# Draghoyns/FLAIR-1

Measured on AMD Instinct MI355X. Metric: 512x512x5 tiles/s (train fwd+bwd), higher is better.
Workload: dtype bf16; 1 GPU; U-Net/ResNet34 5-ch 512x512 13-class train step (fwd + fused CE/argmax/confmat + bwd + SGD), bs=32/GPU, random-init weights; global_batch=32, parallelism=dp1, grad_allreduce=none

## Files before the change

flair-1_amd/csrc/capi.hip:

```cpp
#include <new>
#include <string.h>

#include "../../include/flair_hip.h"
#include "unet.h"
#include "conv_args.h"
#include "parity_pack.h"
#include "segformer.h"
#include "upernet.h"
#include "segformer_ops.h"
#include "swin_ops.h"

using namespace flair;

struct flair_unet { UNet net; flair_unet(int a, int b, int c) : net(a, b, c) {} };
struct flair_segformer {
  SegFormer net;
  flair_segformer(int a, int b, const int* d, const int* h, const int* hd, const int* sr, int dh, int dt) : net(a, b, d, h, hd, sr, dh, dt) {}
};

struct flair_upernet {
  UperNet net;
  flair_upernet(int a, int b, int e, const int* d, const int* h, int hid, const int* ps, int ai, int ac, int dt)
      : net(a, b, e, d, h, hid, ps, ai, ac, dt) {}
};
// ... 605 lines not shown
  if (dtype != DT_F32 && dtype != DT_BF16) return -2;
  return maxpool3x3s2_bwd(dtype, dy, idx, dx, accumulate, N, H, W, C, (hipStream_t)stream, bnr_y, bnr_msc, bnr_msh, bnr_partial);
}
int flair_bn_act(int dtype, const void* y, const float* scale, const float* shift, void* out, int64_t rows, int C, int relu, void* stream) {
  if (!y || !scale || !shift || !out || rows < 1 || C < 1) return -1;
  if (dtype != DT_F32 && dtype != DT_BF16) return -2;
  return bn_act(dtype, y, scale, shift, nullptr, nullptr, nullptr, out, (long)rows, C, relu, (hipStream_t)stream);
}
int flair_bn_act_maxpool(int dtype, const void* y, const float* scale, const float* shift, void* act, void* out, uint8_t* idx, int N,
                         int H, int W, int C, void* stream) {
  if (!y || !scale || !shift || !act || !out || N < 1 || H < 1 || W < 1 || C < 1) return -1;
  if (dtype != DT_F32 && dtype != DT_BF16) return -2;
  return bn_act_maxpool3x3s2(dtype, y, scale, shift, act, out, idx, N, H, W, C, (hipStream_t)stream);
}
int flair_upcat_bwd(int dtype, const void* dcat, void* dx0, int dx0_accumulate, void* dskip, int dskip_accumulate, int N, int H, int W,
                    int C0, int C1, void* stream) {
  if (!dcat || !dx0 || (C1 > 0 && !dskip) || N < 1 || H < 1 || W < 1 || C0 < 1 || C1 < 0) return -1;
  if (dtype != DT_F32 && dtype != DT_BF16) return -2;
  return upcat_bwd(dtype, dcat, dx0, dx0_accumulate, dskip, dskip_accumulate, N, H, W, C0, C1, (hipStream_t)stream);
}
int flair_ew_add(int dtype, void* dst, const void* src, int64_t n, void* stream) {
  if (!dst || !src || n < 1) return -1;
  if (dtype != DT_F32 && dtype != DT_BF16) return -2;
  return ew_add(dtype, dst, src, (long)n, (hipStream_t)stream);
}
int flair_colsum(int dtype, const void* x, int64_t rows, int ld, int C, float* out, void* workspace, size_t wsb, void* stream) {
  if (!x || !out || !workspace || rows < 1 || ld < 1 || C < 1) return -1;
  if (dtype != DT_F32 && dtype != DT_BF16) return -2;
  OpArena ar(workspace, wsb);
  float* partial = (float*)ar.get((size_t)bn_bwd_blocks((long)rows) * ld * 4);
  if (ar.bad) return -100;
  return colsum(dtype, x, (long)rows, ld, C, partial, out, (hipStream_t)stream);
}
int flair_pack_weights(int dtype, const float* params, const flair_pack_desc_t* descs, int n, void* base, void* stream) {
  if (!params || !descs || !base) return -1;
  if ((dtype != DT_F32 && dtype != DT_BF16) || n < 1 || n > PackTable::MAX) return -2;
  PackTable tb;
  tb.n = n;
  for (int i = 0; i < n; ++i) {
    const flair_pack_desc_t& q = descs[i];
    const int taps = q.Rc > 0 ? q.Rc * q.Sc : q.R * q.S;
    if (q.Cout < 1 || q.Cin < 1 || q.R < 1 || q.S < 1 || taps < 1 || (long)taps * q.Cin_p > q.Kpad || q.Cin_p < (q.tf ? q.Cout : q.Cin) ||
        q.rows_pad < (q.tf ? q.Cin : q.Cout) || q.w_off < 0)
      return -2;
    const bool vec = dtype == DT_BF16 && q.R * q.S == 9 &&
                     (q.tf ? ((q.Cin & 31) == 0 && (q.Cout & 31) == 0) : (q.Rc == 0 && (q.Cin & 3) == 0));
    if (vec && (((uintptr_t)params & 15) || (q.w_off & 3))) return -2;
    if (q.Rc > 0 && (q.r0 + (q.Rc - 1) * q.rstep >= q.R || q.s0 + (q.Sc - 1) * q.sstep >= q.S || q.r0 < 0 || q.s0 < 0 || q.rstep < 1 || q.sstep < 1))
      return -2;
    PackDesc& d = tb.d[i];
    memset(&d, 0, sizeof(d));
    d.w_off = (long)q.w_off; d.dst_off = (size_t)q.dst_off; d.Cout = q.Cout; d.Cin = q.Cin; d.R = q.R; d.S = q.S;
    d.Cin_p = q.Cin_p; d.rows_pad = q.rows_pad; d.Kpad = q.Kpad; d.tf = q.tf;
    d.r0 = (unsigned char)q.r0; d.rstep = (unsigned char)q.rstep; d.Rc = (unsigned char)q.Rc;
    d.s0 = (unsigned char)q.s0; d.sstep = (unsigned char)q.sstep; d.Sc = (unsigned char)q.Sc;
  }
  return pack_weights_all(dtype, params, base, tb, (hipStream_t)stream);
}
int flair_pack_weight(int dtype, const float* w_oihw, void* dst, int Cout, int Cin, int R, int S, int Cin_p, int rows_pad, int Kpad,
                      int tf, void* stream) {
  if (!w_oihw || !dst) return -1;
  if (dtype != DT_F32 && dtype != DT_BF16) return -2;
  if (Cout < 1 || Cin < 1 || R < 1 || S < 1 || (long)R * S * Cin_p > Kpad || Cin_p < (tf ? Cout : Cin) || rows_pad < (tf ? Cin : Cout))
    return -2;
  return pack_weight(dtype, w_oihw, dst, Cout, Cin, R, S, Cin_p, rows_pad, Kpad, tf ? 1 : 0, (hipStream_t)stream);
}

int flair_maxpool_forward(int dtype, const void* x, void* y, uint8_t* idx, int N, int H, int W, int C, void* stream) {
  return maxpool3x3s2_fwd(dtype, x, y, idx, N, H, W, C, (hipStream_t)stream);
}
int flair_maxpool_backward(int dtype, const void* dy, const uint8_t* idx, void* dx, int N, int H, int W, int C, void* stream) {
  return maxpool3x3s2_bwd(dtype, dy, idx, dx, 0, N, H, W, C, (hipStream_t)stream);
}
int flair_nchw_to_nhwc(int dtype, const float* x, void* y, int N, int C, int H, int W, int Cpad, void* stream) {
  return nchw_f32_to_nhwc(dtype, x, y, N, C, H, W, Cpad, (hipStream_t)stream);
}
int flair_nhwc_to_nchw(int dtype, const void* x, float* y, int N, int C, int H, int W, int Cpad, void* stream) {
  return nhwc_to_nchw_f32(dtype, x, y, N, C, H, W, Cpad, nullptr, (hipStream_t)stream);
}

#define FLAIR_DT_OK(dt) ((dt) == DT_F32 || (dt) == DT_BF16)
int flair_sf_layernorm(int dtype, const void* x, const float* gamma, const float* beta, void* y, int64_t rows, int C, float eps, void* stream) {
  if (!x || !gamma || !beta || !y || rows < 1 || C < 1) return -1;
  if (!FLAIR_DT_OK(dtype)) return -2;
  return sf_layernorm(dtype, x, gamma, beta, y, (long)rows, C, eps, (hipStream_t)stream);
}
int flair_sf_dwconv3x3_gelu(int dtype, const void* x, const float* w, const float* bias, void* y, int B, int H, int W, int C, void* stream) {
  if (!x || !w || !bias || !y || B < 1 || H < 1 || W < 1 || C < 1) return -1;
  if (!FLAIR_DT_OK(dtype)) return -2;
  return sf_dwconv3x3_gelu(dtype, x, w, bias, y, B, H, W, C, (hipStream_t)stream);
// ... 165 lines not shown
```

flair-1_amd/csrc/misc.hip:

```cpp
#include "ops.h"
#include "prof.h"

namespace flair {

static inline int ew_blocks(long total) {
  long b = (total + 255) / 256;
  if (b > 256 * 16) b = 256 * 16;
  if (b < 1) b = 1;
  return (int)b;
}

template <typename T>
__global__ void maxpool_fwd_kernel(const T* __restrict__ in, T* __restrict__ out, unsigned char* __restrict__ idx,
                                   int N, int H, int W, int C) {
  constexpr int CH = Elem<T>::CH;
  const int Ho = H / 2, Wo = W / 2, cpr = C / CH;
  const int ho = blockIdx.x % Ho, n = blockIdx.x / Ho;
  const unsigned row_items = (unsigned)Wo * cpr;
  for (unsigned it = threadIdx.x; it < row_items; it += blockDim.x) {
    const int cx = (int)(it % (unsigned)cpr), wo = (int)(it / (unsigned)cpr);
    const long i = ((long)blockIdx.x * Wo + wo) * cpr + cx;
    float best[CH];
    unsigned char bi[CH];
#pragma unroll
// ... 338 lines not shown
        }
      }
      __syncthreads();
      for (int e = t; e < 32 * 32 * RSc; e += 256) {
        const int kk = e & 31, rest = e >> 5;
        const int tp = rest % RSc, cc = rest / RSc;
        if (k0 + kk < d.Cout && c0 + cc < d.Cin) {
          const int r = r0 + (tp / Sc) * rstep, q = s0 + (tp % Sc) * sstep;
          const float v = tile[(kk * 32 + cc) * RS + (d.R - 1 - r) * d.S + (d.S - 1 - q) + (kk >> 3)];
          dst[(long)(c0 + cc) * d.Kpad + tp * d.Cin_p + k0 + kk] = Elem<T>::from_f(v);
        }
      }
    }
  } else {
    const long total = (long)d.Cin * d.Cout * RSc;
    for (long i = (long)blockIdx.x * 256 + t; i < total; i += (long)gridDim.x * 256) {
      const int k = (int)(i % d.Cout);
      const long rest = i / d.Cout;
      const int tp = (int)(rest % RSc), c = (int)(rest / RSc);
      const int r = r0 + (tp / Sc) * rstep, q = s0 + (tp % Sc) * sstep;
      dst[(long)c * d.Kpad + tp * d.Cin_p + k] =
          Elem<T>::from_f(w[(((long)k * d.Cin + c) * d.R + (d.R - 1 - r)) * d.S + (d.S - 1 - q)]);
    }
  }
  const int nrows = d.tf ? d.Cin : d.Cout, ncols = d.tf ? d.Cout : d.Cin;
  const long total = (long)d.rows_pad * d.Kpad;
  for (long i = (long)blockIdx.x * 256 + t; i < total; i += (long)gridDim.x * 256) {
    const int row = (int)(i / d.Kpad), kk = (int)(i - (long)row * d.Kpad);
    const int tp = kk / d.Cin_p, c = kk - tp * d.Cin_p;
    if (row >= nrows || tp >= RSc || c >= ncols) dst[i] = Elem<T>::from_f(0.f);
  }
}

int pack_weights_all(int dtype, const float* params, void* base, const PackTable& tb, hipStream_t s) {
  if (tb.n < 1 || tb.n > PackTable::MAX) return -2;
  double bytes = 0;
  for (int i = 0; i < tb.n; ++i) bytes += (double)tb.d[i].Cout * tb.d[i].Cin * tb.d[i].R * tb.d[i].S * 4.0 + (double)tb.d[i].rows_pad * tb.d[i].Kpad * dtype_size(dtype);
  ProfScope ps("pack_weights_all", 0.0, bytes, s);
  dim3 grid(256, tb.n);
  if (dtype == DT_F32)
    hipLaunchKernelGGL(pack_weights_all_kernel<float>, grid, dim3(256), 0, s, params, (unsigned char*)base, tb);
  else
    hipLaunchKernelGGL(pack_weights_all_kernel<bf16_t>, grid, dim3(256), 0, s, params, (unsigned char*)base, tb);
  FLAIR_CHECK_LAUNCH();
  return 0;
}

__global__ void sgd_kernel(float* __restrict__ p, const float* __restrict__ g, long n, float lr) {
  const long n4 = n / 4;
  for (long i = (long)blockIdx.x * blockDim.x + threadIdx.x; i < n4; i += (long)gridDim.x * blockDim.x) {
    float4 a = reinterpret_cast<float4*>(p)[i];
    const float4 b = reinterpret_cast<const float4*>(g)[i];
    a.x -= lr * b.x; a.y -= lr * b.y; a.z -= lr * b.z; a.w -= lr * b.w;
    reinterpret_cast<float4*>(p)[i] = a;
  }
  if (blockIdx.x == 0 && threadIdx.x < (n & 3)) {
    const long i = n4 * 4 + threadIdx.x;
    p[i] -= lr * g[i];
  }
}

__global__ void add_rowvec_kernel(float* __restrict__ x, const float* __restrict__ v, int N, int C, int H, int W) {
  const long total = (long)N * C * H * W;
  for (long i = (long)blockIdx.x * blockDim.x + threadIdx.x; i < total; i += (long)gridDim.x * blockDim.x) {
    const int h = (int)((i / W) % H);
    const int n = (int)(i / ((long)C * H * W));
    x[i] += v[n * H + h];
  }
}

template <typename T>
__global__ void add_rowvec_nhwc_kernel(T* __restrict__ x, const float* __restrict__ v, long nchunks, int row_chunks) {
  constexpr int CH = Elem<T>::CH;
  for (long i = (long)blockIdx.x * blockDim.x + threadIdx.x; i < nchunks; i += (long)gridDim.x * blockDim.x) {
    const float a = v[i / row_chunks];
    float f[CH];
// ... 236 lines not shown
```

flair-1_amd/csrc/ops.h:

```cpp
#pragma once
#include "common.h"
#include "conv_route.h"

namespace flair {

int bn_finalize(const float* partial, int nblk, int C, long count, const float* gamma, const float* beta,
                float* running_mean, float* running_var, float momentum, float eps, float* scale, float* shift,
                float* mean_out, float* invstd_out, hipStream_t s);
int bn_eval_coeffs(int C, const float* gamma, const float* beta, const float* rm, const float* rv, float eps,
                   float* scale, float* shift, hipStream_t s);
int bn_act(int dtype, const void* y, const float* scale, const float* shift, const void* res, const float* rscale,
           const float* rshift, void* out, long rows, int C, int relu, hipStream_t s);
int bn_bwd_blocks(long rows);
int bn_backward(int dtype, const void* dout, const void* out, const void* y, const float* mean, const float* invstd,
                const float* gamma, long rows, int C, float* partial, float* coef, float* dgamma, float* dbeta,
                int accumulate_param, void* dy, void* dres, int dres_accumulate, const float* mscale, const float* mshift,
                int pre_nblk ,
                int premasked , hipStream_t s);

int partial_rows_sum(const float* partial, int nblk, int ncols, float* out, hipStream_t s);
int bn_stats_partial(int dtype, const void* y, long rows, int C, float* partial, float* zeros_ones, hipStream_t s);
int colsum(int dtype, const void* x, long rows, int ld, int C, float* partial, float* out, hipStream_t s);

int maxpool3x3s2_fwd(int dtype, const void* in, void* out, unsigned char* idx, int N, int H, int W, int C, hipStream_t s);
int bn_act_maxpool3x3s2(int dtype, const void* y, const float* scale, const float* shift, void* act, void* out, unsigned char* idx, int N, int H,
                        int W, int C, hipStream_t s);
int maxpool3x3s2_bwd(int dtype, const void* dout, const unsigned char* idx, void* din, int accumulate, int N, int H,
                     int W, int C, hipStream_t s, const void* bnr_y = nullptr, const float* bnr_msc = nullptr,
                     const float* bnr_msh = nullptr, float* bnr_partial = nullptr);
int upcat_bwd(int dtype, const void* dcat, void* dx0, int dx0_accumulate, void* dskip, int dskip_accumulate, int N,
              int H, int W, int C0, int C1, hipStream_t s);
int nchw_f32_to_nhwc(int dtype, const float* in, void* out, int N, int C, int H, int W, int Cp, hipStream_t s);
int nhwc_to_nchw_f32(int dtype, const void* in, float* out, int N, int C, int H, int W, int Cp, float* accumulate_into,
                     hipStream_t s);
int pack_weight(int dtype, const float* w_oihw, void* dst, int Cout, int Cin, int R, int S, int Cin_p, int rows_pad,
                int Kpad, int transpose_flip, hipStream_t s);
struct PackDesc {
  long w_off;
  size_t dst_off;
  int Cout, Cin, R, S, Cin_p, rows_pad, Kpad, tf;
  unsigned char r0, rstep, Rc, s0, sstep, Sc, pad_[2];
};
inline PackDesc pack_desc(long w_off, size_t dst_off, int Cout, int Cin, int R, int Cin_p, int rows_pad, int Kpad, int tf) {
  PackDesc d = {};
  d.w_off = w_off; d.dst_off = dst_off; d.Cout = Cout; d.Cin = Cin; d.R = R; d.S = R;
  d.Cin_p = Cin_p; d.rows_pad = rows_pad; d.Kpad = Kpad; d.tf = tf;
  return d;
}
struct PackTable {
  static constexpr int MAX = 64;
  int n;
  PackDesc d[MAX];
};
int pack_weights_all(int dtype, const float* params, void* base, const PackTable& tb, hipStream_t s);
int sgd_step(float* params, const float* grads, long n, float lr, hipStream_t s);
int add_rowvec_nchw(float* x, const float* v, int N, int C, int H, int W, hipStream_t s);
int add_rowvec_nhwc(int dtype, void* x, const float* v, int N, int H, int W, int C, hipStream_t s);
int add_rowvec_nhwc_to(int dtype, const void* x, const float* v, void* y, int N, int H, int W, int C, hipStream_t s);
int rowvec_grad_nhwc(int dtype, const void* dx, float* dv, int N, int H, int W, int C, hipStream_t s);
int ew_add(int dtype, void* dst, const void* src, long n, hipStream_t s);
int fill_zero(void* p, size_t bytes, hipStream_t s);
int fill_f32(float* p, long n, float v, hipStream_t s);

struct CeArgs {
  const float* logits;
  const void* logits_nhwc = nullptr;
  int logits_dtype = 0, logits_ld = 0;
  const void* labels;
  int label_kind;
  const float* weight;
  int B, C, H, W;
  float* loss;
  float* dlogits_nchw;
  void* dlogits_nhwc;
  int dlogits_dtype, dlogits_ld;
  unsigned char* preds_u8;
  long long* preds_i64;
  int* targets_i32;
  long long* confmat;
  float* workspace;
};
size_t ce_workspace_floats(int B, int H, int W);
int ce_head(const CeArgs& a, hipStream_t s);
constexpr int CE_MAX_BLOCKS = 2048;
struct CeWorkspace { unsigned char* lab8; float* den_partial; float* loss_partial; float* den; };
CeWorkspace ce_workspace_layout(float* workspace, long npix);
int ce_labels(const void* labels, int label_kind, const float* weight, int B, int C, int H, int W, int* targets_i32, float* workspace, hipStream_t s);
int ce_finish(float* workspace, long npix, int nblk, float* loss, hipStream_t s);
// ... 42 lines not shown
```

flair-1_amd/csrc/unet.h:

```cpp
#pragma once
#include <string>
#include <vector>

#include "ops.h"

namespace flair {

struct Act {
  void* p = nullptr;
  int N = 0, H = 0, W = 0, C = 0;
  const float* lz_scale = nullptr;
  const float* lz_shift = nullptr;
  long rows() const { return (long)N * H * W; }
  long elems() const { return rows() * C; }
};

struct ConvDesc {
  std::string name;
  int Cin, Cout, R, S, stride, pad;
  int Cin_p, Cout_p;
  bool bias;
  long w_off = -1, b_off = -1;
  size_t wf = 0, wd = 0;
  int Kpad, rows_f;
// ... 113 lines not shown
  std::vector<hipEvent_t> fork_ev_;
  hipEvent_t join_ev_ = nullptr;
  size_t fork_next_ = 0;
  bool side_pending_ = false;
  Act f5m_;
  float* drows_pending_ = nullptr;
  bool side_init();
  hipStream_t wgrad_stream();
  int side_cus() const;
  void side_join();
 public:
  ~UNet();
 private:
  void* dl_nhwc_ = nullptr;
  void* logits_nhwc_ = nullptr;
  void* const* stage_events_ = nullptr;
  void stage_done(int stage);

  struct GradBuf { void* act; void* g; bool init; };
  int sole_producer(const Act& a) const;
  int residual_producer(const Act& a) const;
  void attach_bn_reduce(ConvArgs& a, const Act& target);
  std::vector<GradBuf> gbufs_;
  const void* acc_src_next_ = nullptr;
  bool bwd_fuse() const;
  void* grad_of(const Act& a, bool* accumulate);
  void* grad_peek(const Act& a);

  size_t plan_bytes(int B, int H, int W, int training);
  void build_table();
  int add_conv(const std::string& name, int cin, int cout, int k, int stride, int pad, bool bias, int stage);
  int add_bn(const std::string& name, int c, int stage);
  void begin(void* ws, size_t ws_bytes, hipStream_t s, bool dry);
  void pack_forward_weights();
  void pack_dgrad_weights();
  int run_unit(int conv, int bn, const Act& in0, const Act& in1, bool up0, bool relu, int res_unit, const Act& res,
               bool materialize, int lazy_cons = -1, bool lazy_up0 = false, const Act* lazy_skip = nullptr);
  bool lazy_into_hg(const Act& y, int cons, bool up0, const Act& skip) const;
  void encoder_fwd_impl(const float* x_nchw);
  void decoder_fwd_impl();
  void head_fwd_impl(float* logits_nchw, const FwdOpts& o);
  void unit_backward(int ui, const void* dout, void* dres, bool dres_acc, bool need_dgrad, void* dx_override,
                     bool upcat = false);
  void head_bwd_impl(const void* dl);
  void decoder_bwd_impl();
  void encoder_bwd_impl();
  void fwd_common_begin(const float* params, float* buffers, int B, int H, int W, int training);
};

}
```

flair-1_amd/csrc/unet.hip:

```cpp
#include <stdlib.h>

#include "unet.h"
#include "conv_args.h"
#include "conv_route.h"
#include "parity_pack.h"
#include "tune.h"

namespace flair {

#define RUN(expr)                         \
  do {                                    \
    if (!dry_ && !err_) {                 \
      int rc__ = (expr);                  \
      if (rc__) err_ = rc__;              \
    }                                     \
  } while (0)

int UNet::add_conv(const std::string& name, int cin, int cout, int k, int stride, int pad, bool bias, int stage) {
  ConvDesc c;
  c.name = name; c.Cin = cin; c.Cout = cout; c.R = k; c.S = k; c.stride = stride; c.pad = pad; c.bias = bias;
  c.Cin_p = (int)round_up(cin, 8);
  c.Cout_p = (int)round_up(cout < 16 ? 16 : cout, 16);
  c.w_off = n_params;
  TensorInfo t;
// ... 121 lines not shown
  return side_;
}

void UNet::side_join() {
  if (!side_pending_ || dry_) return;
  side_pending_ = false;
  if (hipEventRecord(join_ev_, side_) != hipSuccess || hipStreamWaitEvent(s_, join_ev_, 0) != hipSuccess) {
    if (!err_) err_ = -13;
  }
}

void* UNet::alloc(size_t bytes) {
  const size_t off = top_;
  top_ = (size_t)round_up((long)(top_ + bytes), 256);
  if (!dry_ && top_ > cap_) { if (!err_) err_ = -100; return base_; }
  return base_ + off;
}

Act UNet::alloc_act(int N, int H, int W, int C) {
  Act a;
  a.N = N; a.H = H; a.W = W; a.C = C;
  a.p = alloc((size_t)a.elems() * dtype_size(dtype));
  return a;
}

void UNet::begin(void* ws, size_t ws_bytes, hipStream_t s, bool dry) {
  base_ = dry ? (unsigned char*)0x100000 : (unsigned char*)ws;
  cap_ = ws_bytes; top_ = 0; dry_ = dry; err_ = 0; s_ = s;
  units_.clear();
  gbufs_.clear();
  packed_d_ = false;
  dl_nhwc_ = nullptr;
  logits_nhwc_ = nullptr;
  for (auto& c : convs) {
    c.wf = top_; alloc((size_t)c.rows_f * c.Kpad * dtype_size(dtype));
  }
  for (auto& c : convs) {
    c.wd = top_; alloc((size_t)c.rows_d * c.Kpad_d * dtype_size(dtype));
  }
  for (auto& c : convs) {
    if (!c.parity_dgrad()) continue;
    for (int cls = 0, kg; cls < 4; ++cls) {
      parity_class_geom(dtype, c.Cout_p, cls, kg, c.Kpad_cls[cls]);
      c.wd_cls[cls] = top_; alloc((size_t)c.rows_d * c.Kpad_cls[cls] * dtype_size(dtype));
    }
  }
}

void UNet::pack_forward_weights() {
  PackTable tb;
  tb.n = 0;
  for (auto& c : convs) tb.d[tb.n++] = pack_desc(c.w_off, c.wf, c.Cout, c.Cin, c.R, c.Cin_p, c.rows_f, c.Kpad, 0);
  RUN(pack_weights_all(dtype, params_, base_, tb, s_));
}

void UNet::pack_dgrad_weights() {
  if (packed_d_) return;
  packed_d_ = true;
  PackTable tb;
  tb.n = 0;
  for (size_t i = 1; i < convs.size(); ++i) {
    auto& c = convs[i];
    const PackDesc full = tb.d[tb.n++] = pack_desc(c.w_off, c.wd, c.Cout, c.Cin, c.R, c.Cout_p, c.rows_d, c.Kpad_d, 1);
    if (c.parity_dgrad()) {
      for (int cls = 0; cls < 4; ++cls) tb.d[tb.n++] = parity_class_pack(full, cls, c.wd_cls[cls], c.Kpad_cls[cls]);
    }
  }
  RUN(pack_weights_all(dtype, params_, base_, tb, s_));
}

void* UNet::grad_of(const Act& a, bool* accumulate) {
  for (auto& g : gbufs_)
    if (g.act == a.p) { *accumulate = g.init; g.init = true; return g.g; }
  GradBuf g;
  g.act = a.p;
  g.g = alloc((size_t)a.elems() * dtype_size(dtype));
  g.init = true;
  *accumulate = false;
  gbufs_.push_back(g);
  return g.g;
}

void* UNet::grad_peek(const Act& a) {
  for (auto& g : gbufs_)
    if (g.act == a.p) return g.g;
  return nullptr;
}

static ConvInput conv_input(const Act& in0, const Act& in1, bool up0) {
  return ConvInput{in0.p, in1.p, in0.C, in1.p ? in1.C : 0, up0 ? 1 : 0, in0.N, in0.H, in0.W};
}

static void fill_conv_args(ConvArgs& a, int dtype, const ConvDesc& c, const Act& in0, const Act& in1, bool up0, void* y, const void* wpacked) {
  conv_fwd_args(a, dtype, conv_input(in0, in1, up0), c.R, c.stride, c.pad, c.Cout);
  a.w = wpacked;
  a.out = y; a.out_ld = c.Cout_p;
  a.in_scale = in0.lz_scale; a.in_shift = in0.lz_shift;
}

bool UNet::lazy_into_hg(const Act& y, int cons, bool up0, const Act& skip) const {
  if (!training_ || !tune("FLAIR_LAZY_HG", 1)) return false;
// ... 159 lines not shown
    b.out = nullptr; b.preds_u8 = preds; b.maxprob_f32 = maxprob;
    if (conv_halo_preds_ok(dtype, b)) {
      logits_nhwc_ = nullptr;
      RUN(launch_conv(dtype, b, s_));
      return;
    }
  }
  RUN(launch_conv(dtype, a, s_));
  if (preds && !dry_)
    RUN(softmax_argmax_nhwc(logits_nhwc_, dtype, c.Cout_p, dec_out_.rows(), c.Cout, preds, nullptr, maxprob, s_));
}

int FwdOpts::refusal(int training, bool fp32_logits, int H, int W) const {
  if ((maxprob && !preds) || (drows && !rows)) return -1;
  if (ce.labels && (!ce.loss || !ce.ws || ce.kind < 0 || ce.kind > 3)) return -1;
  if (ce.labels && (preds || training || fp32_logits)) return -15;
  if (rows && training && !drows) return -16;
  if (drows && !training) return -17;
  if ((H % 32) || (W % 32)) return -10;
  return 0;
}

int UNet::forward(const float* params, float* buffers, const float* x_nchw, float* logits_nchw, int B, int H, int W,
                  int training, void* ws, size_t ws_bytes, hipStream_t s, const FwdOpts& o) {
  if (const int rc = o.refusal(training, logits_nchw != nullptr, H, W)) return rc;
  f5m_ = Act(); drows_pending_ = nullptr;
  reuse_ = o.reuse_constants && !training && last_valid_ && ws == last_ws_ && params == last_params_ && buffers == last_buffers_ &&
           B == last_B_ && H == last_H_ && W == last_W_;
  begin(ws, ws_bytes, s, false);
  fwd_common_begin(params, buffers, B, H, W, training);
  const int lazy_env = tune("FLAIR_LAZY_BN", 1);
  lazy_ok_ = lazy_env != 0;
  lazy_max_c_ = lazy_env >= 2 ? 32 : 16;
  if (!reuse_) pack_forward_weights();
  encoder_fwd_impl(x_nchw);
  if (o.rows && !training) RUN(add_rowvec_nhwc(dtype, f_[5].p, o.rows, f_[5].N, f_[5].H, f_[5].W, f_[5].C, s_));
  const Act f5 = f_[5];
  if (o.rows && training) {
    f5m_ = alloc_act(f5.N, f5.H, f5.W, f5.C);
    RUN(add_rowvec_nhwc_to(dtype, f5.p, o.rows, f5m_.p, f5.N, f5.H, f5.W, f5.C, s_));
    f_[5] = f5m_;
    drows_pending_ = o.drows;
  }
  decoder_fwd_impl();
  f_[5] = f5;
  head_fwd_impl(logits_nchw, o);
  fwd_top_ = top_;
  reuse_ = false;
  last_valid_ = !training && !err_;
  last_ws_ = ws; last_params_ = params; last_buffers_ = buffers; last_B_ = B; last_H_ = H; last_W_ = W;
  return err_;
}

int UNet::encoder_forward(const float* params, float* buffers, const float* x_nchw, float* const feats[5], int B, int H,
                          int W, int training, void* ws, size_t ws_bytes, hipStream_t s) {
  invalidate_reuse();
  f5m_ = Act(); drows_pending_ = nullptr;
  if ((H % 32) || (W % 32)) return -10;
  begin(ws, ws_bytes, s, false);
  fwd_common_begin(params, buffers, B, H, W, training);
  lazy_ok_ = false;
  pack_forward_weights();
  encoder_fwd_impl(x_nchw);
  for (int i = 0; i < 5; ++i) {
    const Act& f = f_[i + 1];
    RUN(nhwc_to_nchw_f32(dtype, f.p, feats[i], f.N, f.C, f.H, f.W, f.C, nullptr, s_));
  }
// ... 431 lines not shown
```

flair-1_amd/flair_amd/_lib.py:

```python
from __future__ import annotations

import ctypes as C
import os

import torch

_HERE = os.path.dirname(os.path.abspath(__file__))
LIB_PATH = os.environ.get("FLAIR_HIP_LIB") or os.path.join(_HERE, "libflair_hip.so")

_lib = None

vp, i32, i64, f32, sz = C.c_void_p, C.c_int, C.c_int64, C.c_float, C.c_size_t

PROTOTYPES = {
    "flair_strerror": (C.c_char_p, [i32]),
    "flair_version": (i32, []),
    "flair_unet_create": (i32, [C.POINTER(vp), i32, i32, i32]),
    "flair_unet_destroy": (None, [vp]),
    "flair_unet_param_count": (i64, [vp]),
    "flair_unet_buffer_count": (i64, [vp]),
    "flair_unet_num_tensors": (i32, [vp]),
    "flair_unet_tensor_info": (i32, [vp, i32, C.c_char_p, i32, C.POINTER(i64), C.POINTER(i32), C.POINTER(i64),
                                     C.POINTER(i32), C.POINTER(i32)]),
    "flair_unet_stage_range": (i32, [vp, i32, C.POINTER(i64), C.POINTER(i64)]),
# ... 17 lines not shown
    "flair_jaccard": (i32, [vp, i32, vp, vp, vp, vp]),
    "flair_confmat_masks": (i32, [vp, vp, i64, i32, i32, vp, vp]),
    "flair_feed_tiles": (i32, [vp, vp, vp, i32, i32, i32, i32, C.POINTER(i32), i32, i32, C.POINTER(C.c_double),
                               C.POINTER(C.c_double), i32, vp, vp, vp]),
    "flair_detect_convert": (i32, [vp, i32, i32, i32, i32, i32, vp, vp]),
    "flair_gather_tiles": (i32, [vp, i32, i32, i32, vp, i32, i32, C.POINTER(i32), i32, i32, C.POINTER(C.c_double),
                                 C.POINTER(C.c_double), vp, vp]),
    "flair_detect_stitch": (i32, [vp, i32, i32, i32, i32, i32, vp, vp, i32, i32, vp]),
    "flair_sgd_step": (i32, [vp, vp, i64, f32, vp]),
    "flair_add_rowvec_nchw": (i32, [vp, vp, i32, i32, i32, i32, vp]),
    "flair_add_rowvec_nhwc": (i32, [i32, vp, vp, i32, i32, i32, i32, vp]),
    "flair_add_rowvec_nhwc_to": (i32, [i32, vp, vp, vp, i32, i32, i32, i32, vp]),
    "flair_rowvec_grad_nhwc": (i32, [i32, vp, vp, i32, i32, i32, i32, vp]),
    "flair_conv2d_workspace_bytes": (sz, [i32, i32, i32, i32, i32, i32, i32, i32, i32, i32, i32]),
    "flair_conv2d_forward": (i32, [i32, vp, vp, i32, i32, i32, i32, i32, i32, vp, vp, i32, i32, i32, i32, vp, vp, vp,
                                   vp, sz, vp]),
    "flair_conv2d_backward": (i32, [i32, vp, i32, i32, i32, i32, vp, i32, i32, i32, i32, vp, vp, vp, vp, sz, vp]),
    "flair_conv2d_ex_workspace_bytes": (sz, [vp]),
    "flair_conv2d_ex": (i32, [vp, vp, sz, vp]),
    "flair_conv2d_ex_grid_rows": (i32, [vp]),
    "flair_conv2d_wgrad_ex_workspace_bytes": (sz, [vp]),
    "flair_conv2d_wgrad_ex": (i32, [vp, vp, sz, vp]),
    "flair_bn_workspace_bytes": (sz, [i64, i32]),
    "flair_bn_relu_forward": (i32, [i32, vp, i64, i32, vp, vp, vp, vp, i32, vp, i32, vp, vp, vp, vp, sz, vp]),
    "flair_bn_relu_backward": (i32, [i32, vp, vp, vp, i64, i32, vp, vp, vp, i32, vp, vp, vp, vp, vp, sz, vp]),
    "flair_bn_backward_ex": (i32, [vp, vp, sz, vp]),
    "flair_maxpool_backward_ex": (i32, [i32, vp, vp, vp, i32, i32, i32, i32, i32, vp, vp, vp, vp, vp]),
    "flair_bn_act": (i32, [i32, vp, vp, vp, vp, i64, i32, i32, vp]),
    "flair_bn_act_maxpool": (i32, [i32, vp, vp, vp, vp, vp, vp, i32, i32, i32, i32, vp]),
    "flair_upcat_bwd": (i32, [i32, vp, vp, i32, vp, i32, i32, i32, i32, i32, i32, vp]),
    "flair_ew_add": (i32, [i32, vp, vp, i64, vp]),
    "flair_colsum": (i32, [i32, vp, i64, i32, i32, vp, vp, sz, vp]),
    "flair_pack_weights": (i32, [i32, vp, vp, i32, vp, vp]),
    "flair_pack_weight": (i32, [i32, vp, vp, i32, i32, i32, i32, i32, i32, i32, i32, vp]),
    "flair_maxpool_forward": (i32, [i32, vp, vp, vp, i32, i32, i32, i32, vp]),
    "flair_maxpool_backward": (i32, [i32, vp, vp, vp, i32, i32, i32, i32, vp]),
    "flair_nchw_to_nhwc": (i32, [i32, vp, vp, i32, i32, i32, i32, i32, vp]),
    "flair_nhwc_to_nchw": (i32, [i32, vp, vp, i32, i32, i32, i32, i32, vp]),
    "flair_sf_layernorm": (i32, [i32, vp, vp, vp, vp, i64, i32, f32, vp]),
    "flair_sf_dwconv3x3_gelu": (i32, [i32, vp, vp, vp, vp, i32, i32, i32, i32, vp]),
    "flair_sf_bilinear_nhwc": (i32, [i32, vp, vp, i32, i32, i32, i32, i32, i32, i32, vp]),
    "flair_sf_bilinear_nchw_f32": (i32, [vp, vp, i64, i32, i32, i32, i32, vp]),
    "flair_sf_slice_cols": (i32, [i32, vp, i32, i32, i32, i64, vp, vp]),
    "flair_sf_fuse_bias": (i32, [vp, i32, vp, vp, vp, vp, vp, vp, vp, vp]),
    "flair_sf_upsample_sum_bn_relu": (i32, [i32, vp, vp, vp, vp, vp, vp, vp, i32, i32, i32, i32, vp]),
    "flair_sf_ffn_fused_ok": (i32, [i32, i32, i32, i32]),
    "flair_sf_ffn_dw_pack": (i32, [vp, vp, vp, i32, vp]),
    "flair_sf_ffn_fused": (i32, [vp, vp, vp, vp, vp, vp, vp, vp, vp, i32, i32, i32, i32, f32, vp, vp, vp, vp]),
    "flair_sf_head_fused_ok": (i32, [i32, i32, i32, i32, i32, i32]),
    "flair_sf_head_wint": (i32, [vp, vp]),
    "flair_sf_head_fused": (i32, [vp, vp, vp, vp, vp, vp, vp, vp, vp, vp, vp, i32, i32, i32, i32, i32, vp]),
    "flair_sf_attention": (i32, [i32, vp, vp, vp, vp, i32, i32, i32, i32, i32, vp]),
    "flair_swin_window_attention": (i32, [i32, vp, vp, vp, vp, i32, i32, i32, i32, i32, i32, vp]),
    "flair_swin_layernorm": (i32, [i32, vp, vp, vp, vp, i64, i32, i32, f32, vp]),
    "flair_swin_patch_merge_ln": (i32, [i32, vp, vp, vp, vp, i32, i32, i32, i32, f32, vp]),
    "flair_swin_adaptive_avgpool": (i32, [i32, vp, i32, vp, i32, i32, i32, i32, i32, vp]),
    "flair_swin_bilinear_add": (i32, [i32, vp, vp, i32, i32, i32, i32, i32, i32, vp]),
    "flair_profile_start": (i32, [i32]),
    "flair_profile_stop": (i32, []),
    "flair_profile_kernel": (i32, [i32, C.c_char_p, i32, C.POINTER(C.c_double), C.POINTER(i64), C.POINTER(C.c_double),
                                   C.POINTER(C.c_double)]),
    "flair_metadata_mlp_forward": (i32, [vp, vp, vp, vp, vp, vp, vp, i32, vp]),
    "flair_metadata_mlp_backward": (i32, [vp, vp, vp, vp, vp, vp, vp, i32, vp, vp, vp, vp]),
    "flair_detect_stitch_preds": (i32, [vp, vp, i32, i32, i32, vp, vp, i32, i32, vp]),
    "flair_detect_blend_accum": (i32, [vp, i32, i32, i32, i32, vp, vp, i32, i32, i32, i32, vp, i32, i32, vp]),
    "flair_detect_blend_flush": (i32, [vp, i32, i32, i32, i32, vp, i32, i32, vp]),
# ... 130 lines not shown
```

include/flair_hip.h:

```cpp
#ifndef FLAIR_HIP_H
#define FLAIR_HIP_H
#include <stddef.h>
#include <stdint.h>

#ifdef __cplusplus
extern "C" {
#endif

#define FLAIR_DT_F32 0
#define FLAIR_DT_BF16 1

const char* flair_strerror(int code);
int flair_version(void);

typedef struct flair_unet flair_unet_t;
int flair_unet_create(flair_unet_t** out, int in_channels, int classes, int dtype);
void flair_unet_destroy(flair_unet_t* h);
int64_t flair_unet_param_count(const flair_unet_t* h);
int64_t flair_unet_buffer_count(const flair_unet_t* h);
int flair_unet_num_tensors(const flair_unet_t* h);
int flair_unet_tensor_info(const flair_unet_t* h, int i, char* name, int name_cap, int64_t shape[4], int* ndim,
                           int64_t* offset, int* kind, int* stage);
int flair_unet_stage_range(const flair_unet_t* h, int stage, int64_t* begin, int64_t* end);
int64_t flair_unet_workspace_bytes(flair_unet_t* h, int B, int H, int W, int training);
// ... 149 lines not shown
                           void* stream);
typedef struct flair_bn_bwd_ex {
  int dtype;
  const void* dout; const void* out; const void* y;
  const float* mean; const float* invstd; const float* gamma;
  int64_t rows; int C;
  float* partial; int pre_nblk; int premasked;
  const float* mscale; const float* mshift;
  float* dgamma; float* dbeta; int accumulate_param;
  void* dy; void* dres; int dres_accumulate;
  float* coef;
} flair_bn_bwd_ex_t;
int flair_bn_backward_ex(const flair_bn_bwd_ex_t* p, void* workspace, size_t workspace_bytes, void* stream);
int flair_maxpool_forward(int dtype, const void* x, void* y, uint8_t* idx, int N, int H, int W, int C, void* stream);
int flair_maxpool_backward(int dtype, const void* dy, const uint8_t* idx, void* dx, int N, int H, int W, int C,
                           void* stream);
int flair_maxpool_backward_ex(int dtype, const void* dy, const uint8_t* idx, void* dx, int accumulate, int N, int H, int W, int C,
                              const void* bnr_y, const float* bnr_msc, const float* bnr_msh, float* bnr_partial, void* stream);
int flair_bn_act(int dtype, const void* y, const float* scale, const float* shift, void* out, int64_t rows, int C, int relu,
                 void* stream);
int flair_bn_act_maxpool(int dtype, const void* y, const float* scale, const float* shift, void* act, void* out, uint8_t* idx, int N,
                         int H, int W, int C, void* stream);
int flair_upcat_bwd(int dtype, const void* dcat, void* dx0, int dx0_accumulate, void* dskip, int dskip_accumulate, int N, int H, int W,
                    int C0, int C1, void* stream);
int flair_ew_add(int dtype, void* dst, const void* src, int64_t n, void* stream);
int flair_colsum(int dtype, const void* x, int64_t rows, int ld, int C, float* out, void* workspace, size_t workspace_bytes,
                 void* stream);
typedef struct flair_pack_desc {
  int64_t w_off; uint64_t dst_off;
  int Cout, Cin, R, S, Cin_p, rows_pad, Kpad, tf;
  int r0, rstep, Rc, s0, sstep, Sc;
} flair_pack_desc_t;
int flair_pack_weights(int dtype, const float* params, const flair_pack_desc_t* descs, int n, void* base, void* stream);
int flair_pack_weight(int dtype, const float* w_oihw, void* dst, int Cout, int Cin, int R, int S, int Cin_p, int rows_pad, int Kpad,
                      int tf, void* stream);
int flair_nchw_to_nhwc(int dtype, const float* x_nchw, void* y_nhwc, int N, int C, int H, int W, int Cpad, void* stream);
int flair_nhwc_to_nchw(int dtype, const void* x_nhwc, float* y_nchw, int N, int C, int H, int W, int Cpad, void* stream);

int flair_sf_layernorm(int dtype, const void* x, const float* gamma, const float* beta, void* y, int64_t rows, int C, float eps,
                       void* stream);
int flair_sf_dwconv3x3_gelu(int dtype, const void* x, const float* w, const float* bias, void* y, int B, int H, int W, int C,
                            void* stream);
int flair_sf_bilinear_nhwc(int dtype, const void* x, void* y, int B, int h, int w, int C, int H, int W, int ld, void* stream);
int flair_sf_bilinear_nchw_f32(const float* x, float* y, int64_t planes, int h, int w, int H, int W, void* stream);
int flair_sf_slice_cols(int dtype, const float* src, int ld, int col0, int ncols, int64_t rows, void* dst, void* stream);
int flair_sf_fuse_bias(const float* wf, int D, const float* b3, const float* b2, const float* b1, const float* b0,
                       const float* scale, const float* shift, float* shift2, void* stream);
int flair_sf_upsample_sum_bn_relu(int dtype, const void* g0, const void* g1, const void* g2, const void* g3, const float* scale,
                                  const float* shift2, void* z, int B, int H, int W, int D, void* stream);
int flair_sf_ffn_fused_ok(int dtype, int C, int H, int W);
int flair_sf_ffn_dw_pack(const float* w, const float* b, float* out, int nch, void* stream);
int flair_sf_ffn_fused(const void* x, const float* ln_g, const float* ln_b, const void* w1, const float* b1, const float* dwp,
                       const void* w2, const float* b2, void* out, int B, int H, int W, int C, float eps, const float* ln2_g,
                       const float* ln2_b, void* out_ln, void* stream);
int flair_sf_head_fused_ok(int dtype, int H, int W, int C0, int D, int labels);
int flair_sf_head_wint(void* wint_bf16_128x96, void* stream);
int flair_sf_head_fused(const void* f0, const void* w0, const void* g1, const void* g2, const void* g3, const void* wint,
                        const float* scale, const float* shift2, const void* wc, const float* bc, float* out, int B, int H, int W,
                        int D, int labels, void* stream);
int flair_sf_attention(int dtype, const void* q, const void* k, const void* v, void* out, int B, int N, int Nk, int hidden,
                       int kv_ld, void* stream);
int flair_swin_window_attention(int dtype, const void* qkv, const float* qkv_bias, const float* table, void* out, int B, int H,
                                int W, int C, int heads, int shift, void* stream);
int flair_swin_layernorm(int dtype, const void* x, const float* gamma, const float* beta, void* y, int64_t rows, int C, int ld,
                         float eps, void* stream);
int flair_swin_patch_merge_ln(int dtype, const void* x, const float* gamma, const float* beta, void* y, int B, int H, int W, int C,
// ... 54 lines not shown
```

Baseline: 2821 tiles/s.

## Fuse forward, dgrad and parity-class weight packing into one tiled kernel

```diff
diff --git a/flair-1_amd/csrc/capi.hip b/flair-1_amd/csrc/capi.hip
--- a/flair-1_amd/csrc/capi.hip
+++ b/flair-1_amd/csrc/capi.hip
@@ -661,30 +661,80 @@
   if (ar.bad) return -100;
   return colsum(dtype, x, (long)rows, ld, C, partial, out, (hipStream_t)stream);
 }
+static int pack_desc_from_c(int dtype, const float* params, const flair_pack_desc_t& q, PackDesc& d) {
+  const int taps = q.Rc > 0 ? q.Rc * q.Sc : q.R * q.S;
+  if (q.Cout < 1 || q.Cin < 1 || q.R < 1 || q.S < 1 || taps < 1 || (long)taps * q.Cin_p > q.Kpad || q.Cin_p < (q.tf ? q.Cout : q.Cin) ||
+      q.rows_pad < (q.tf ? q.Cin : q.Cout) || q.w_off < 0)
+    return -2;
+  const bool vec = dtype == DT_BF16 && q.R * q.S == 9 &&
+                   (q.tf ? ((q.Cin & 31) == 0 && (q.Cout & 31) == 0) : (q.Rc == 0 && (q.Cin & 3) == 0));
+  if (vec && (((uintptr_t)params & 15) || (q.w_off & 3))) return -2;
+  if (q.Rc > 0 && (q.r0 + (q.Rc - 1) * q.rstep >= q.R || q.s0 + (q.Sc - 1) * q.sstep >= q.S || q.r0 < 0 || q.s0 < 0 || q.rstep < 1 || q.sstep < 1))
+    return -2;
+  memset(&d, 0, sizeof(d));
+  d.w_off = (long)q.w_off; d.dst_off = (size_t)q.dst_off; d.Cout = q.Cout; d.Cin = q.Cin; d.R = q.R; d.S = q.S;
+  d.Cin_p = q.Cin_p; d.rows_pad = q.rows_pad; d.Kpad = q.Kpad; d.tf = q.tf;
+  d.r0 = (unsigned char)q.r0; d.rstep = (unsigned char)q.rstep; d.Rc = (unsigned char)q.Rc;
+  d.s0 = (unsigned char)q.s0; d.sstep = (unsigned char)q.sstep; d.Sc = (unsigned char)q.Sc;
+  return 0;
+}
 int flair_pack_weights(int dtype, const float* params, const flair_pack_desc_t* descs, int n, void* base, void* stream) {
   if (!params || !descs || !base) return -1;
   if ((dtype != DT_F32 && dtype != DT_BF16) || n < 1 || n > PackTable::MAX) return -2;
   PackTable tb;
   tb.n = n;
-  for (int i = 0; i < n; ++i) {
-    const flair_pack_desc_t& q = descs[i];
-    const int taps = q.Rc > 0 ? q.Rc * q.Sc : q.R * q.S;
-    if (q.Cout < 1 || q.Cin < 1 || q.R < 1 || q.S < 1 || taps < 1 || (long)taps * q.Cin_p > q.Kpad || q.Cin_p < (q.tf ? q.Cout : q.Cin) ||
-        q.rows_pad < (q.tf ? q.Cin : q.Cout) || q.w_off < 0)
-      return -2;
-    const bool vec = dtype == DT_BF16 && q.R * q.S == 9 &&
-                     (q.tf ? ((q.Cin & 31) == 0 && (q.Cout & 31) == 0) : (q.Rc == 0 && (q.Cin & 3) == 0));
-    if (vec && (((uintptr_t)params & 15) || (q.w_off & 3))) return -2;
-    if (q.Rc > 0 && (q.r0 + (q.Rc - 1) * q.rstep >= q.R || q.s0 + (q.Sc - 1) * q.sstep >= q.S || q.r0 < 0 || q.s0 < 0 || q.rstep < 1 || q.sstep < 1))
-      return -2;
-    PackDesc& d = tb.d[i];
-    memset(&d, 0, sizeof(d));
-    d.w_off = (long)q.w_off; d.dst_off = (size_t)q.dst_off; d.Cout = q.Cout; d.Cin = q.Cin; d.R = q.R; d.S = q.S;
-    d.Cin_p = q.Cin_p; d.rows_pad = q.rows_pad; d.Kpad = q.Kpad; d.tf = q.tf;
-    d.r0 = (unsigned char)q.r0; d.rstep = (unsigned char)q.rstep; d.Rc = (unsigned char)q.Rc;
-    d.s0 = (unsigned char)q.s0; d.sstep = (unsigned char)q.sstep; d.Sc = (unsigned char)q.Sc;
-  }
+  for (int i = 0; i < n; ++i)
+    if (const int rc = pack_desc_from_c(dtype, params, descs[i], tb.d[i])) return rc;
   return pack_weights_all(dtype, params, base, tb, (hipStream_t)stream);
+}
+int flair_pack_layers(int dtype, const float* params, const flair_pack_desc_t* descs, int n_descs, void* base, void* stream) {
+  if (!params || !descs || !base) return -1;
+  if ((dtype != DT_F32 && dtype != DT_BF16) || n_descs < 1 || n_descs > PackTable::MAX) return -2;
+  LayerPackTable tb;
+  tb.n = 0;
+  bool used[PackTable::MAX] = {};
+  for (int i = 0; i < n_descs; ++i) {
+    if (used[i] || descs[i].tf || descs[i].Rc > 0) continue;
+    PackDesc f, full, cls[4];
+    if (const int rc = pack_desc_from_c(dtype, params, descs[i], f)) return rc;
+    if (f.R != f.S) return -2;
+    used[i] = true;
+    int have_full = 0, have_cls = 0;
+    for (int k = 0; k < n_descs; ++k) {
+      const flair_pack_desc_t& q = descs[k];
+      if (used[k] || q.w_off != descs[i].w_off) continue;
+      if (!q.tf || q.Cout != f.Cout || q.Cin != f.Cin || q.R != f.R || q.S != f.S) return -2;
+      used[k] = true;
+      if (q.Rc == 0) {
+        if (have_full++) return -2;
+        if (const int rc = pack_desc_from_c(dtype, params, q, full)) return rc;
+      }
+    }
+    if (have_full) {
+      for (int k = 0; k < n_descs; ++k) {
+        const flair_pack_desc_t& q = descs[k];
+        if (q.w_off != descs[i].w_off || !q.tf || q.Rc == 0) continue;
+        PackDesc d;
+        if (const int rc = pack_desc_from_c(dtype, params, q, d)) return rc;
+        int cl = -1;
+        for (int c = 0; c < 4; ++c) {
+          const PackDesc e = parity_class_pack(full, c, d.dst_off, d.Kpad);
+          if (f.R == 3 && e.Rc == d.Rc && e.r0 == d.r0 && e.rstep == d.rstep && e.Sc == d.Sc && e.s0 == d.s0 && e.sstep == d.sstep &&
+              d.Cin_p == full.Cin_p && d.rows_pad == full.rows_pad)
+            cl = c;
+        }
+        if (cl < 0 || (have_cls & (1 << cl))) return -2;
+        have_cls |= 1 << cl;
+        cls[cl] = d;
+      }
+      if (have_cls != 0 && have_cls != 15) return -2;
+    }
+    if (tb.n == LayerPackTable::MAX) return -2;
+    tb.j[tb.n++] = layer_pack_job(f, have_full ? &full : nullptr, have_cls ? cls : nullptr);
+  }
+  for (int i = 0; i < n_descs; ++i)
+    if (!used[i]) return -2;
+  return pack_layers_all(dtype, params, base, tb, (hipStream_t)stream);
 }
 int flair_pack_weight(int dtype, const float* w_oihw, void* dst, int Cout, int Cin, int R, int S, int Cin_p, int rows_pad, int Kpad,
                       int tf, void* stream) {
diff --git a/flair-1_amd/csrc/misc.hip b/flair-1_amd/csrc/misc.hip
--- a/flair-1_amd/csrc/misc.hip
+++ b/flair-1_amd/csrc/misc.hip
@@ -394,6 +394,112 @@
   }
 }
 
+template <typename T>
+__device__ __forceinline__ void pack_layers_zero_pad(T* __restrict__ dst, int rows_pad, int Kpad, int Cin_p, int nrows, int ncols, int ntaps) {
+  const long total = (long)rows_pad * Kpad;
+  for (long i = (long)blockIdx.x * 256 + threadIdx.x; i < total; i += (long)gridDim.x * 256) {
+    const int row = (int)(i / Kpad), kk = (int)(i - (long)row * Kpad);
+    const int tp = kk / Cin_p, c = kk - tp * Cin_p;
+    if (row >= nrows || tp >= ntaps || c >= ncols) dst[i] = Elem<T>::from_f(0.f);
+  }
+}
+
+template <typename T>
+__global__ __launch_bounds__(256) void pack_layers_kernel(const float* __restrict__ params, unsigned char* __restrict__ base,
+                                                          const LayerPackTable tb) {
+  __shared__ float tile[32 * (32 * 9 + 1)];
+  const LayerPackJob& d = tb.j[blockIdx.y];
+  const int t = threadIdx.x;
+  const float* __restrict__ w = params + d.w_off;
+  T* __restrict__ df = reinterpret_cast<T*>(base + d.wf);
+  const int R = d.R, RS = R * R;
+  if (RS > 9) {
+    const int nitems = d.Cout * d.Cin;
+    for (int item = blockIdx.x * 256 + t; item < nitems; item += gridDim.x * 256) {
+      const int k = item / d.Cin, c = item - k * d.Cin;
+      const float* src = w + (long)item * RS;
+      T* drow = df + (long)k * d.Kpad_f + c;
+      for (int tp = 0; tp < RS; ++tp) drow[tp * d.Cin_pf] = Elem<T>::from_f(src[tp]);
+    }
+  } else {
+    const int LDK = 32 * RS + 1;
+    const int ct = (d.Cin + 31) / 32, kt = (d.Cout + 31) / 32;
+    const bool vec = ((d.Cin * RS) & 3) == 0 && (d.w_off & 3) == 0;
+    T* __restrict__ dd = reinterpret_cast<T*>(base + d.wd);
+    for (int tl = blockIdx.x; tl < ct * kt; tl += gridDim.x) {
+      const int c0 = (tl % ct) * 32, k0 = (tl / ct) * 32;
+      const int nk = d.Cout - k0 < 32 ? d.Cout - k0 : 32, nc = d.Cin - c0 < 32 ? d.Cin - c0 : 32;
+      const int len = nc * RS;
+      __syncthreads();
+      if (vec) {
+        const int nq = len >> 2;
+        for (int e = t; e < nk * nq; e += 256) {
+          const int kk = e / nq, j = e - kk * nq;
+          const long off = ((long)(k0 + kk) * d.Cin + c0) * RS + 4 * j;
+          const float4 a = *reinterpret_cast<const float4*>(w + off);
+          float* tr = tile + kk * LDK + 4 * j;
+          tr[0] = a.x; tr[1] = a.y; tr[2] = a.z; tr[3] = a.w;
+        }
+      } else {
+        for (int e = t; e < nk * len; e += 256) {
+          const int kk = e / len, j = e - kk * len;
+          const long off = ((long)(k0 + kk) * d.Cin + c0) * RS + j;
+          tile[kk * LDK + j] = w[off];
+        }
+      }
+      __syncthreads();
+      constexpr int LW = sizeof(T) == 2 ? 16 : 32;
+      constexpr int PER = sizeof(T) == 2 ? 2 : 1;
+      const int lf = t & (LW - 1), ls = t / LW;
+      auto put = [&](T* p, const float* tr, int hi_stride, bool hi_ok) {
+        if constexpr (sizeof(T) == 2) {
+          const unsigned lo = f32_to_bf16(tr[0]), hi = hi_ok ? (unsigned)f32_to_bf16(tr[hi_stride]) : 0u;
+          *reinterpret_cast<unsigned*>(p) = lo | (hi << 16);
+        } else {
+          *p = Elem<T>::from_f(tr[0]);
+        }
+      };
+      {
+        const int cc = PER * lf;
+        if (cc < nc)
+          for (int kk = ls; kk < nk; kk += 256 / LW) {
+            const float* tr = tile + kk * LDK + cc * RS;
+            T* drow = df + (long)(k0 + kk) * d.Kpad_f + c0 + cc;
+            for (int tp = 0; tp < RS; ++tp) put(drow + tp * d.Cin_pf, tr + tp, RS, cc + 1 < nc);
+          }
+      }
+      const int ncopies = d.has_d ? (d.has_cls ? 5 : 1) : 0;
+      const int kk = PER * lf;
+      if (kk < nk)
+        for (int cp = 0; cp < ncopies; ++cp) {
+          T* __restrict__ dst = cp == 0 ? dd : reinterpret_cast<T*>(base + d.wc[cp - 1]);
+          const int Kpad = cp == 0 ? d.Kpad_d : d.Kpad_c[cp - 1];
+          const int py = (cp - 1) >> 1, px = (cp - 1) & 1;
+          const int Rc = cp == 0 ? R : (py ? 2 : 1), Sc = cp == 0 ? R : (px ? 2 : 1);
+          const int r0 = cp == 0 ? 0 : (py ? 0 : 1), s0 = cp == 0 ? 0 : (px ? 0 : 1), step = cp == 0 ? 1 : 2;
+          for (int cc = ls; cc < nc; cc += 256 / LW) {
+            const float* tr = tile + kk * LDK + cc * RS;
+            T* drow = dst + (long)(c0 + cc) * Kpad + k0 + kk;
+            for (int ri = 0; ri < Rc; ++ri)
+              for (int si = 0; si < Sc; ++si) {
+                const int r = r0 + ri * step, q = s0 + si * step;
+                put(drow + (ri * Sc + si) * d.Cout_pd, tr + (R - 1 - r) * R + (R - 1 - q), LDK, kk + 1 < nk);
+              }
+          }
+        }
+    }
+  }
+  if (d.pad_mask & 1) pack_layers_zero_pad<T>(df, d.rows_f, d.Kpad_f, d.Cin_pf, d.Cout, d.Cin, RS);
+  if (d.has_d) {
+    if (d.pad_mask & 2) pack_layers_zero_pad<T>(reinterpret_cast<T*>(base + d.wd), d.rows_d, d.Kpad_d, d.Cout_pd, d.Cin, d.Cout, RS);
+    if (d.has_cls)
+      for (int cls = 0; cls < 4; ++cls)
+        if (d.pad_mask & (4 << cls))
+          pack_layers_zero_pad<T>(reinterpret_cast<T*>(base + d.wc[cls]), d.rows_d, d.Kpad_c[cls], d.Cout_pd, d.Cin, d.Cout,
+                               ((cls >> 1) ? 2 : 1) * ((cls & 1) ? 2 : 1));
+  }
+}
+
 int pack_weights_all(int dtype, const float* params, void* base, const PackTable& tb, hipStream_t s) {
   if (tb.n < 1 || tb.n > PackTable::MAX) return -2;
   double bytes = 0;
@@ -404,6 +510,58 @@
     hipLaunchKernelGGL(pack_weights_all_kernel<float>, grid, dim3(256), 0, s, params, (unsigned char*)base, tb);
   else
     hipLaunchKernelGGL(pack_weights_all_kernel<bf16_t>, grid, dim3(256), 0, s, params, (unsigned char*)base, tb);
+  FLAIR_CHECK_LAUNCH();
+  return 0;
+}
+
+LayerPackJob layer_pack_job(const PackDesc& f, const PackDesc* dg, const PackDesc* cls) {
+  LayerPackJob j = {};
+  j.w_off = f.w_off; j.wf = f.dst_off;
+  j.Cout = f.Cout; j.Cin = f.Cin; j.R = f.R;
+  j.Cin_pf = f.Cin_p; j.rows_f = f.rows_pad; j.Kpad_f = f.Kpad;
+  const int RS = f.R * f.S;
+  if (f.rows_pad != f.Cout || f.Cin_p != f.Cin || f.Kpad != RS * f.Cin_p) j.pad_mask |= 1;
+  if (dg) {
+    j.has_d = 1; j.wd = dg->dst_off;
+    j.Cout_pd = dg->Cin_p; j.rows_d = dg->rows_pad; j.Kpad_d = dg->Kpad;
+    if (dg->rows_pad != f.Cin || dg->Cin_p != f.Cout || dg->Kpad != RS * dg->Cin_p) j.pad_mask |= 2;
+    if (cls) {
+      j.has_cls = 1;
+      for (int c = 0; c < 4; ++c) {
+        j.wc[c] = cls[c].dst_off; j.Kpad_c[c] = cls[c].Kpad;
+        if (dg->rows_pad != f.Cin || dg->Cin_p != f.Cout || cls[c].Kpad != cls[c].Rc * cls[c].Sc * dg->Cin_p) j.pad_mask |= 4 << c;
+      }
+    }
+  }
+  return j;
+}
+
+int pack_layers_all(int dtype, const float* params, void* base, const LayerPackTable& tb, hipStream_t s) {
+  if (tb.n < 1 || tb.n > LayerPackTable::MAX) return -2;
+  double bytes = 0;
+  for (int i = 0; i < tb.n; ++i) {
+    const LayerPackJob& j = tb.j[i];
+    if (j.w_off < 0 || j.Cout < 1 || j.Cin < 1 || j.R < 1) return -2;
+    if (j.R > 3 && j.has_d) return -2;
+    if (j.has_cls && (j.R != 3 || !j.has_d)) return -2;
+    if (((j.Cin * j.R * j.R) & 3) == 0 && (j.w_off & 3) == 0 && ((uintptr_t)params & 15)) return -2;
+    if (dtype == DT_BF16) {
+      bool even = !((j.Cin_pf | j.Kpad_f) & 1) && !(j.wf & 3);
+      if (j.has_d) even = even && !((j.Cout_pd | j.Kpad_d) & 1) && !(j.wd & 3);
+      if (j.has_cls) for (int c = 0; c < 4; ++c) even = even && !(j.Kpad_c[c] & 1) && !(j.wc[c] & 3);
+      if (!even || ((uintptr_t)base & 3)) return -2;
+    }
+    const size_t es = dtype_size(dtype);
+    bytes += (double)j.Cout * j.Cin * j.R * j.R * 4.0 + (double)j.rows_f * j.Kpad_f * es;
+    if (j.has_d) bytes += (double)j.rows_d * j.Kpad_d * es;
+    if (j.has_cls) for (int c = 0; c < 4; ++c) bytes += (double)j.rows_d * j.Kpad_c[c] * es;
+  }
+  ProfScope ps("pack_layers", 0.0, bytes, s);
+  dim3 grid(256, tb.n);
+  if (dtype == DT_F32)
+    hipLaunchKernelGGL(pack_layers_kernel<float>, grid, dim3(256), 0, s, params, (unsigned char*)base, tb);
+  else
+    hipLaunchKernelGGL(pack_layers_kernel<bf16_t>, grid, dim3(256), 0, s, params, (unsigned char*)base, tb);
   FLAIR_CHECK_LAUNCH();
   return 0;
 }
diff --git a/flair-1_amd/csrc/ops.h b/flair-1_amd/csrc/ops.h
--- a/flair-1_amd/csrc/ops.h
+++ b/flair-1_amd/csrc/ops.h
@@ -54,6 +54,23 @@
 };
 int pack_weights_all(int dtype, const float* params, void* base, const PackTable& tb, hipStream_t s);
 int sgd_step(float* params, const float* grads, long n, float lr, hipStream_t s);
+struct LayerPackJob {
+  long w_off;
+  size_t wf, wd, wc[4];
+  int Cout, Cin, R;
+  int Cin_pf, rows_f, Kpad_f;
+  int Cout_pd, rows_d, Kpad_d;
+  int Kpad_c[4];
+  int has_d, has_cls;
+  int pad_mask;
+};
+LayerPackJob layer_pack_job(const PackDesc& fwd, const PackDesc* dgrad, const PackDesc* cls4);
+struct LayerPackTable {
+  static constexpr int MAX = 48;
+  int n;
+  LayerPackJob j[MAX];
+};
+int pack_layers_all(int dtype, const float* params, void* base, const LayerPackTable& tb, hipStream_t s);
 int add_rowvec_nchw(float* x, const float* v, int N, int C, int H, int W, hipStream_t s);
 int add_rowvec_nhwc(int dtype, void* x, const float* v, int N, int H, int W, int C, hipStream_t s);
 int add_rowvec_nhwc_to(int dtype, const void* x, const float* v, void* y, int N, int H, int W, int C, hipStream_t s);
diff --git a/flair-1_amd/csrc/unet.h b/flair-1_amd/csrc/unet.h
--- a/flair-1_amd/csrc/unet.h
+++ b/flair-1_amd/csrc/unet.h
@@ -169,8 +169,10 @@
   int add_conv(const std::string& name, int cin, int cout, int k, int stride, int pad, bool bias, int stage);
   int add_bn(const std::string& name, int c, int stage);
   void begin(void* ws, size_t ws_bytes, hipStream_t s, bool dry);
+  size_t layout_weight_arena();
   void pack_forward_weights();
   void pack_dgrad_weights();
+  void pack_all_weights();
   int run_unit(int conv, int bn, const Act& in0, const Act& in1, bool up0, bool relu, int res_unit, const Act& res,
                bool materialize, int lazy_cons = -1, bool lazy_up0 = false, const Act* lazy_skip = nullptr);
   bool lazy_into_hg(const Act& y, int cons, bool up0, const Act& skip) const;
diff --git a/flair-1_amd/csrc/unet.hip b/flair-1_amd/csrc/unet.hip
--- a/flair-1_amd/csrc/unet.hip
+++ b/flair-1_amd/csrc/unet.hip
@@ -177,25 +177,32 @@
   packed_d_ = false;
   dl_nhwc_ = nullptr;
   logits_nhwc_ = nullptr;
-  for (auto& c : convs) {
-    c.wf = top_; alloc((size_t)c.rows_f * c.Kpad * dtype_size(dtype));
-  }
-  for (auto& c : convs) {
-    c.wd = top_; alloc((size_t)c.rows_d * c.Kpad_d * dtype_size(dtype));
-  }
+  top_ = layout_weight_arena();
+  if (!dry_ && top_ > cap_) err_ = -100;
+}
+
+size_t UNet::layout_weight_arena() {
+  size_t top = 0;
+  auto take = [&](size_t bytes) { const size_t off = top; top = (size_t)round_up((long)(top + bytes), 256); return off; };
+  for (auto& c : convs) c.wf = take((size_t)c.rows_f * c.Kpad * dtype_size(dtype));
+  for (auto& c : convs) c.wd = take((size_t)c.rows_d * c.Kpad_d * dtype_size(dtype));
   for (auto& c : convs) {
     if (!c.parity_dgrad()) continue;
     for (int cls = 0, kg; cls < 4; ++cls) {
       parity_class_geom(dtype, c.Cout_p, cls, kg, c.Kpad_cls[cls]);
-      c.wd_cls[cls] = top_; alloc((size_t)c.rows_d * c.Kpad_cls[cls] * dtype_size(dtype));
-    }
-  }
-}
+      c.wd_cls[cls] = take((size_t)c.rows_d * c.Kpad_cls[cls] * dtype_size(dtype));
+    }
+  }
+  return top;
+}
+
+static PackDesc fwd_pack_desc(const ConvDesc& c) { return pack_desc(c.w_off, c.wf, c.Cout, c.Cin, c.R, c.Cin_p, c.rows_f, c.Kpad, 0); }
+static PackDesc dgrad_pack_desc(const ConvDesc& c) { return pack_desc(c.w_off, c.wd, c.Cout, c.Cin, c.R, c.Cout_p, c.rows_d, c.Kpad_d, 1); }
 
 void UNet::pack_forward_weights() {
   PackTable tb;
   tb.n = 0;
-  for (auto& c : convs) tb.d[tb.n++] = pack_desc(c.w_off, c.wf, c.Cout, c.Cin, c.R, c.Cin_p, c.rows_f, c.Kpad, 0);
+  for (auto& c : convs) tb.d[tb.n++] = fwd_pack_desc(c);
   RUN(pack_weights_all(dtype, params_, base_, tb, s_));
 }
 
@@ -206,12 +213,29 @@
   tb.n = 0;
   for (size_t i = 1; i < convs.size(); ++i) {
     auto& c = convs[i];
-    const PackDesc full = tb.d[tb.n++] = pack_desc(c.w_off, c.wd, c.Cout, c.Cin, c.R, c.Cout_p, c.rows_d, c.Kpad_d, 1);
+    const PackDesc full = tb.d[tb.n++] = dgrad_pack_desc(c);
     if (c.parity_dgrad()) {
       for (int cls = 0; cls < 4; ++cls) tb.d[tb.n++] = parity_class_pack(full, cls, c.wd_cls[cls], c.Kpad_cls[cls]);
     }
   }
   RUN(pack_weights_all(dtype, params_, base_, tb, s_));
+}
+
+void UNet::pack_all_weights() {
+  LayerPackTable tb;
+  tb.n = 0;
+  for (size_t i = 0; i < convs.size(); ++i) {
+    const ConvDesc& c = convs[i];
+    const PackDesc f = fwd_pack_desc(c);
+    if (i == 0) { tb.j[tb.n++] = layer_pack_job(f, nullptr, nullptr); continue; }
+    const PackDesc full = dgrad_pack_desc(c);
+    PackDesc cls[4];
+    if (c.parity_dgrad())
+      for (int k = 0; k < 4; ++k) cls[k] = parity_class_pack(full, k, c.wd_cls[k], c.Kpad_cls[k]);
+    tb.j[tb.n++] = layer_pack_job(f, &full, c.parity_dgrad() ? cls : nullptr);
+  }
+  RUN(pack_layers_all(dtype, params_, base_, tb, s_));
+  packed_d_ = true;
 }
 
 void* UNet::grad_of(const Act& a, bool* accumulate) {
@@ -437,7 +461,8 @@
   const int lazy_env = tune("FLAIR_LAZY_BN", 1);
   lazy_ok_ = lazy_env != 0;
   lazy_max_c_ = lazy_env >= 2 ? 32 : 16;
-  if (!reuse_) pack_forward_weights();
+  if (training && tune("FLAIR_PACK_FUSED", 1)) pack_all_weights();
+  else if (!reuse_) pack_forward_weights();
   encoder_fwd_impl(x_nchw);
   if (o.rows && !training) RUN(add_rowvec_nhwc(dtype, f_[5].p, o.rows, f_[5].N, f_[5].H, f_[5].W, f_[5].C, s_));
   const Act f5 = f_[5];
diff --git a/flair-1_amd/flair_amd/_lib.py b/flair-1_amd/flair_amd/_lib.py
--- a/flair-1_amd/flair_amd/_lib.py
+++ b/flair-1_amd/flair_amd/_lib.py
@@ -73,6 +73,7 @@
     "flair_ew_add": (i32, [i32, vp, vp, i64, vp]),
     "flair_colsum": (i32, [i32, vp, i64, i32, i32, vp, vp, sz, vp]),
     "flair_pack_weights": (i32, [i32, vp, vp, i32, vp, vp]),
+    "flair_pack_layers": (i32, [i32, vp, vp, i32, vp, vp]),
     "flair_pack_weight": (i32, [i32, vp, vp, i32, i32, i32, i32, i32, i32, i32, i32, vp]),
     "flair_maxpool_forward": (i32, [i32, vp, vp, vp, i32, i32, i32, i32, vp]),
     "flair_maxpool_backward": (i32, [i32, vp, vp, vp, i32, i32, i32, i32, vp]),
diff --git a/include/flair_hip.h b/include/flair_hip.h
--- a/include/flair_hip.h
+++ b/include/flair_hip.h
@@ -205,6 +205,7 @@
   int r0, rstep, Rc, s0, sstep, Sc;
 } flair_pack_desc_t;
 int flair_pack_weights(int dtype, const float* params, const flair_pack_desc_t* descs, int n, void* base, void* stream);
+int flair_pack_layers(int dtype, const float* params, const flair_pack_desc_t* descs, int n_descs, void* base, void* stream);
 int flair_pack_weight(int dtype, const float* w_oihw, void* dst, int Cout, int Cin, int R, int S, int Cin_p, int rows_pad, int Kpad,
                       int tf, void* stream);
 int flair_nchw_to_nhwc(int dtype, const float* x_nchw, void* y_nhwc, int N, int C, int H, int W, int Cpad, void* stream);
```

Measured after the change: 2841 tiles/s, median of 6. No clear change (+0.7%).
